# IIT-PAVIS/Acoustic-Image-Generation

Measured on AMD Instinct MI355X. Metric: train-step images/sec, higher is better.
Workload: dtype f32

## Files before the change

### acoustic-image-generation_amd/csrc/igemm.hip

```cpp
#include "wgrad_split3_kernel.hpp"
#include "wgrad_tap_kernel.hpp"
#include "igemm_split3d_kernel.hpp"
#include "igemm_split3dp_kernel.hpp"
#include "igemm_split3r_kernel.hpp"
#include "igemm_split3h_kernel.hpp"
#include "skinny_kernel.hpp"
#include <cstdlib>
#include <algorithm>
#include <type_traits>

namespace acimg {

__global__ __launch_bounds__(256) void igemm_splitk_reduce_kernel(const float* slab, int splits,
                                                                  int M, int Ngemm, int slab_ld,
                                                                  const EpiParams e) {
    const long idx = (long)blockIdx.x * 256 + threadIdx.x;
    const long total = (long)M * Ngemm;
    if (idx >= total) return;
    const int m = (int)(idx / Ngemm);
    const int n = (int)(idx - (long)m * Ngemm);
    float v = 0.f;
    for (int z = 0; z < splits; ++z) v += slab[((long)z * M + m) * slab_ld + n];
    if (n >= e.Nstore) return;
    int cn, pixoff, r, q, oh, ow;
    epi_col(e, n, cn, pixoff, r, q);
    const long rp = epi_row_pix(e, m, oh, ow);
    if (epi_lands(e, oh, ow, r, q)) epi_store(e, rp + pixoff, cn, v);
}

__global__ __launch_bounds__(256) void subpixel_weights_kernel(const float* w, int R, int S, int Ko, int Kin, int ldw, int U,
                                                               int V, float* wc, int total) {
    const int idx = blockIdx.x * 256 + threadIdx.x;
    if (idx >= total) return;
    const int ncol = 4 * Ko;
    const int row = idx / ncol, col = idx - row * ncol;
    const int kin = row % Kin, tap = row / Kin;
    const int up = tap / V, vp = tap - up * V;
    const int cls = col / Ko, ko = col - cls * Ko;
    const int a = cls >> 1, b = cls & 1;
    const int r = a + 2 * (U - 1 - up), q = b + 2 * (V - 1 - vp);
    wc[idx] = (r < R && q < S) ? w[((long)(r * S + q) * Ko + ko) * ldw + kin] : 0.f;
}

template <int BMO, int BN, int WGM = 2>
__global__ __launch_bounds__(256) void wgrad_f32_kernel(const WgradParams p) {
    constexpr int BKR = 16;
    constexpr int LDA_S = BMO + 4;
    constexpr int LDB_S = BN + 4;
    constexpr int WGN = 4 / WGM;
    constexpr int WTM = BMO / WGM, WTN = BN / WGN;
    static_assert(WTM % 16 == 0 && WTN % 16 == 0, "wave tile");
    constexpr int TM = WTM / 16, TN = WTN / 16;
    constexpr int AQ = BMO / 4;
    constexpr int ARPP = 256 / AQ;
    constexpr int NA = (BKR + ARPP - 1) / ARPP;
    constexpr int BQ = BN / 4;
    constexpr int BRPP = 256 / BQ;
    constexpr int NB = (BKR + BRPP - 1) / BRPP;

    __shared__ __attribute__((aligned(16))) float As[BKR * LDA_S];
    __shared__ __attribute__((aligned(16))) float Bs[BKR * LDB_S];

    const int tid = threadIdx.x;
    const int lane = tid & 63, wid = tid >> 6;
    const int wm = wid / WGN, wn = wid % WGN;
    const int li = lane & 15, g = lane >> 4;
    const int kk0 = blockIdx.x * BMO, n0 = blockIdx.y * BN;

    const int m_begin = blockIdx.z * p.rows_per_split;
    const int m_end = min(p.M, m_begin + p.rows_per_split);

    const int aq = tid % AQ;
    const int arow0 = tid / AQ;
    const int kk = kk0 + aq * 4;
    const bool kk_ok = kk < p.KK;
    const bool kk_ones = p.db_out != nullptr && kk == p.KK;
    int r = 0, s = 0, c = 0;
    if (kk_ok) {
        const int tap = kk / p.C;
        c = kk - tap * p.C;
        r = tap / p.S;
        s = tap - r * p.S;
    }
    const int bq = tid % BQ;
    const int brow0 = tid / BQ;
    const int nb = n0 + bq * 4;
    const bool nb_ok = nb < p.Nld;
    const int ohw = p.OH * p.OW;

    int x_img[NA], x_oh[NA], x_ow[NA];
#pragma unroll
    for (int j = 0; j < NA; ++j) {
        const int m = m_begin + arow0 + j * ARPP;
        x_img[j] = m / ohw;
        const int rem = m - x_img[j] * ohw;
        x_oh[j] = rem / p.OW;
        x_ow[j] = rem - x_oh[j] * p.OW;
    }

    float4 ra[NA], rb[NB];
    auto load_tiles = [&](int mb) {
#pragma unroll
        for (int j = 0; j < NA; ++j) {
            const int row = arow0 + j * ARPP;
            const int m = mb + row;
            float4 v = make_float4(0.f, 0.f, 0.f, 0.f);
            if (row < BKR && kk_ones && m < m_end) v.x = 1.f;
            if (row < BKR && kk_ok && m < m_end) {
                const int ih = x_oh[j] * p.stride - p.pad_t + r;
                const int iw = x_ow[j] * p.stride - p.pad_l + s;
                if ((unsigned)ih < (unsigned)p.H && (unsigned)iw < (unsigned)p.W)
                    v = *reinterpret_cast<const float4*>(
                        p.X + ((long)(x_img[j] * p.H + ih) * p.W + iw) * p.ldx + c);
            }
            ra[j] = v;
            x_ow[j] += BKR;
            while (x_ow[j] >= p.OW) {
                x_ow[j] -= p.OW;
                if (++x_oh[j] == p.OH) {
                    x_oh[j] = 0;
                    ++x_img[j];
                }
            }
        }
#pragma unroll
        for (int j = 0; j < NB; ++j) {
            const int row = brow0 + j * BRPP;
            const int m = mb + row;
            float4 v = make_float4(0.f, 0.f, 0.f, 0.f);
            if (row < BKR && nb_ok && m < m_end)
                v = *reinterpret_cast<const float4*>(p.G + (long)m * p.ldg + nb);
            rb[j] = v;
        }
    };
    auto store_tiles = [&]() {
#pragma unroll
        for (int j = 0; j < NA; ++j) {
            const int row = arow0 + j * ARPP;
            if (row < BKR) *reinterpret_cast<float4*>(&As[row * LDA_S + aq * 4]) = ra[j];
        }
#pragma unroll
        for (int j = 0; j < NB; ++j) {
            const int row = brow0 + j * BRPP;
            if (row < BKR) *reinterpret_cast<float4*>(&Bs[row * LDB_S + bq * 4]) = rb[j];
        }
    };

    f32x4 acc[TM][TN];
#pragma unroll
    for (int i = 0; i < TM; ++i)
#pragma unroll
        for (int j = 0; j < TN; ++j) acc[i][j] = f32x4{0.f, 0.f, 0.f, 0.f};

    if (m_begin < m_end) {
        load_tiles(m_begin);
        store_tiles();
    }
    __syncthreads();
    for (int mb = m_begin; mb < m_end; mb += BKR) {
        const bool more = (mb + BKR) < m_end;
        if (more) load_tiles(mb + BKR);
        float af[TM][4], bf[TN][4];
#pragma unroll
        for (int t = 0; t < 4; ++t) {
#pragma unroll
            for (int i = 0; i < TM; ++i) af[i][t] = As[(4 * g + t) * LDA_S + wm * WTM + i * 16 + li];
#pragma unroll
            for (int j = 0; j < TN; ++j) bf[j][t] = Bs[(4 * g + t) * LDB_S + wn * WTN + j * 16 + li];
        }
#pragma unroll
        for (int t = 0; t < 4; ++t)
#pragma unroll
            for (int i = 0; i < TM; ++i)
#pragma unroll
                for (int j = 0; j < TN; ++j)
                    acc[i][j] = __builtin_amdgcn_mfma_f32_16x16x4f32(af[i][t], bf[j][t], acc[i][j], 0, 0, 0);
        __syncthreads();
        if (more) {
            store_tiles();
            __syncthreads();
        }
    }

    float* out = p.out + (long)blockIdx.z * p.KK * p.ldo;
#pragma unroll
    for (int i = 0; i < TM; ++i)
#pragma unroll
        for (int rg = 0; rg < 4; ++rg) {
            const int row = kk0 + wm * WTM + i * 16 + g * 4 + rg;
            if (row > p.KK || (row == p.KK && p.db_out == nullptr)) continue;
            float* dst = row < p.KK ? out + (long)row * p.ldo : p.db_out + (long)blockIdx.z * p.ldo;
#pragma unroll
            for (int j = 0; j < TN; ++j) {
                const int n = n0 + wn * WTN + j * 16 + li;
                if (n < p.Ngemm) dst[n] = acc[i][j][rg];
            }
        }
}

__global__ __launch_bounds__(256) void slab_reduce_kernel(const float* slab, int splits, long rows,
                                                          int ncols, int ld, float* out, int nb1,
                                                          const float* slab2, float* out2) {
    long bid = blockIdx.x;
    if (bid >= nb1) {
        bid -= nb1;
        slab = slab2;
        out = out2;
        rows = 1;
    }
    const long idx = bid * 256 + threadIdx.x;
    if (idx >= rows * ncols) return;
    const long row = idx / ncols;
    const int col = (int)(idx - row * ncols);
    float v = 0.f;
    for (int z = 0; z < splits; ++z) v += slab[((long)z * rows + row) * ld + col];
    out[row * ld + col] = v;
}

template <int OUTS>
__global__ __launch_bounds__(256) void slab_reduce_wide_kernel(const float* slab, int splits, long rows,
                                                               int ncols, int ld, float* out, int nb1,
                                                               const float* slab2, float* out2) {
    constexpr int NG = 256 / OUTS;
    __shared__ float red[NG][OUTS];
    const int ol = threadIdx.x % OUTS, rg = threadIdx.x / OUTS;
    long bid = blockIdx.x;
    if (bid >= nb1) {
        bid -= nb1;
        slab = slab2;
        out = out2;
        rows = 1;
    }
    const long idx = bid * OUTS + ol;
    const bool ok = idx < rows * ncols;
    const long row = ok ? idx / ncols : 0;
    const int col = ok ? (int)(idx - row * ncols) : 0;
    const float* src = slab + row * ld + col;
    const long zs = rows * ld;
    float v0 = 0.f, v1 = 0.f, v2 = 0.f, v3 = 0.f;
    if (ok) {
        int z = rg;
        for (; z + 3 * NG < splits; z += 4 * NG) {
            v0 += src[(long)z * zs];
            v1 += src[(long)(z + NG) * zs];
            v2 += src[(long)(z + 2 * NG) * zs];
            v3 += src[(long)(z + 3 * NG) * zs];
        }
        for (; z < splits; z += NG) v0 += src[(long)z * zs];
    }
    red[rg][ol] = (v0 + v1) + (v2 + v3);
    __syncthreads();
    if (rg == 0 && ok) {
        float t = 0.f;
#pragma unroll
        for (int i = 0; i < NG; ++i) t += red[i][ol];
        out[row * ld + col] = t;
    }
}
static void launch_slab_reduce_wide(const float* slab, int splits, long rows, int ncols, int ld, float* out, const float* slab2,
                                    float* out2, hipStream_t st) {
    const long total = rows * ncols;
    if (total <= 4096) {
        const int nb1 = (int)cdiv(total, 8), nb2 = out2 ? cdiv(ncols, 8) : 0;
        hipLaunchKernelGGL(slab_reduce_wide_kernel<8>, dim3(nb1 + nb2), dim3(256), 0, st, slab, splits, rows, ncols, ld, out, nb1,
                           slab2, out2);
    } else {
        const int nb1 = (int)cdiv(total, 32), nb2 = out2 ? cdiv(ncols, 32) : 0;
        hipLaunchKernelGGL(slab_reduce_wide_kernel<32>, dim3(nb1 + nb2), dim3(256), 0, st, slab, splits, rows, ncols, ld, out, nb1,
                           slab2, out2);
    }
}

__global__ __launch_bounds__(256) void tapconv_pack_kernel(const float* w, int taps, int C, int K, int ldw,
                                                           float* wt, int ldwt) {
    const long idx = (long)blockIdx.x * 256 + threadIdx.x;
    const int TK = taps * K;
    if (idx >= (long)C * TK) return;
    const int c = (int)(idx / TK), n = (int)(idx - (long)c * TK);
    const int tap = n / K, k = n - tap * K;
    wt[(long)c * ldwt + n] = w[((long)tap * C + c) * ldw + k];
}

__global__ __launch_bounds__(256) void tapconv_unpack_kernel(const float* dwt, int ldwt, int taps, int C, int K,
                                                             int ldw, const float* w, float decay, float* dw) {
    const long idx = (long)blockIdx.x * 256 + threadIdx.x;
    if (idx >= (long)taps * C * K) return;
    const int k = (int)(idx % K);
    const long tc = idx / K;
    const int c = (int)(tc % C), tap = (int)(tc / C);
    float v = dwt[(long)c * ldwt + tap * K + k];
    if (w) v = fmaf(decay, w[tc * ldw + k], v);
    dw[tc * ldw + k] = v;
}

constexpr int TG_PPB = 32;
__global__ __launch_bounds__(256) void tapconv_gather_kernel(const float* z, int ldz, int H, int W, int R, int S,
                                                             int K, int OH, int OW, long Mout, float* y, int ldy,
                                                             float* stats, int stats_ld) {
    extern __shared__ __attribute__((aligned(16))) float tg_smem[];
    const int ppb = TG_PPB;
    const long m0 = (long)blockIdx.x * ppb;
    for (int e = threadIdx.x; e < ppb * K; e += 256) {
        const int pl = e / K, k = e - pl * K;
        const long m = m0 + pl;
// ... 1674 lines not shown
    float* Y; int ldy, nout;
    const float* bias; const float* res; int ldres; const float* mask; int ldmask;
    float* stats; int stats_ld;
    int tiles_x, tiles_y; long tiles;
};

template <typename TR, int TERMS, int CIN, int NOUT, int MODE>
__global__ __launch_bounds__(512, 1) void conv_halo16_kernel(const ConvHaloParams p) {
    typedef typename TR::V8 V8;
    constexpr int TH = TERMS == 1 ? 8 : 4, TW = 32, XH = TH + 2, XWV = TW + 2, XW = 36;
    constexpr int PITCH = CIN * 2 + 16;
    constexpr int XPL = XH * XW * PITCH;
    constexpr int KTOT = 9 * CIN;
    constexpr int WROW = KTOT * 2 + 16;
    constexpr int WPL = NOUT * WROW;
    constexpr int NPL = TERMS == 3 ? 2 : 1;
    constexpr int MT = TERMS == 1 ? 2 : 1;
    constexpr int NT = NOUT / 16;
    constexpr int NXL = (XH * XWV * (CIN / 4) + 511) / 512;
    extern __shared__ __attribute__((aligned(16))) float ch16_smem[];
    char* const xl = reinterpret_cast<char*>(ch16_smem);
    char* const wl = xl + NPL * XPL;
    const int tid = threadIdx.x, lane = tid & 63, wid = tid >> 6;
    const int li = lane & 15, g = lane >> 4;
    const int jrow = TERMS == 1 ? wid : wid >> 1;
    const int mcol0 = TERMS == 1 ? 0 : (wid & 1) * 16;

    for (int i = tid; i < NPL * NOUT * (KTOT / 8); i += 512) {
        const int ch = i % (KTOT / 8), r2 = i / (KTOT / 8);
        const int n = r2 % NOUT, pl = r2 / NOUT;
        const uint4 v = *reinterpret_cast<const uint4*>(p.Wimg + (size_t)pl * p.w_lo_off + ((size_t)n * KTOT + ch * 8) * 2);
        *reinterpret_cast<uint4*>(wl + pl * WPL + n * WROW + ch * 16) = v;
    }

    float4 rx[NXL];
    unsigned okm = 0;
    const float4 asc = p.a_scale ? *reinterpret_cast<const float4*>(p.a_scale + (tid % (CIN / 4)) * 4) : make_float4(1.f, 1.f, 1.f, 1.f);
    const float4 ash = p.a_scale ? *reinterpret_cast<const float4*>(p.a_shift + (tid % (CIN / 4)) * 4) : make_float4(0.f, 0.f, 0.f, 0.f);
    auto load_tile = [&](long tile) {
        okm = 0;
        const int tx = (int)(tile % p.tiles_x);
        const long t2 = tile / p.tiles_x;
        const int ty = (int)(t2 % p.tiles_y);
        const long img = t2 / p.tiles_y;
        const float* xi = p.X + img * p.H * p.W * p.ldx;
#pragma unroll
        for (int k = 0; k < NXL; ++k) {
            const int i = tid + 512 * k;
            const int c4 = i % (CIN / 4), pix = i / (CIN / 4);
            const int row = pix / XWV, col = pix - row * XWV;
            const int iy = ty * TH + row - 1, ix = tx * TW + col - 1;
            float4 v = make_float4(0.f, 0.f, 0.f, 0.f);
            if (row < XH && (unsigned)iy < (unsigned)p.H && (unsigned)ix < (unsigned)p.W) {
                v = *reinterpret_cast<const float4*>(xi + ((long)iy * p.W + ix) * p.ldx + c4 * 4);
                okm |= 1u << k;
            }
            rx[k] = v;
        }
    };
    auto store_tile = [&]() {
#pragma unroll
        for (int k = 0; k < NXL; ++k) {
            const int i = tid + 512 * k;
            const int c4 = i % (CIN / 4), pix = i / (CIN / 4);
            const int row = pix / XWV, col = pix - row * XWV;
            if (row < XH) {
                const int off = (row * XW + col) * PITCH + c4 * 8;
                uint2 hi, lo;
                split4<TR>(p.a_scale && ((okm >> k) & 1u) ? affine_relu4(rx[k], asc, ash, p.a_relu != 0) : rx[k], hi, lo);
                *reinterpret_cast<uint2*>(xl + off) = hi;
                if (TERMS == 3) *reinterpret_cast<uint2*>(xl + XPL + off) = lo;
            }
        }
    };

    f32x4 s1[NT], s2[NT];
#pragma unroll
    for (int n = 0; n < NT; ++n) s1[n] = s2[n] = f32x4{0.f, 0.f, 0.f, 0.f};
    f32x4 bv[NT];
#pragma unroll
    for (int n = 0; n < NT; ++n)
        bv[n] = (MODE == 0 && p.bias) ? *reinterpret_cast<const f32x4*>(p.bias + n * 16 + 4 * g) : f32x4{0.f, 0.f, 0.f, 0.f};

    const int a_base = (jrow * XW + mcol0 + li) * PITCH + g * 16;
    const int b_base = li * WROW + g * 16;

    long tile = blockIdx.x;
    if (tile < p.tiles) load_tile(tile);
    for (; tile < p.tiles; tile += gridDim.x) {
        __syncthreads();
        store_tile();
        __syncthreads();
        const int tx = (int)(tile % p.tiles_x);
        const long t2 = tile / p.tiles_x;
        const int ty = (int)(t2 % p.tiles_y);
        const long img = t2 / p.tiles_y;
        if (tile + gridDim.x < p.tiles) load_tile(tile + gridDim.x);
        f32x4 acc[MT][NT];
#pragma unroll
        for (int m = 0; m < MT; ++m)
#pragma unroll
            for (int n = 0; n < NT; ++n) acc[m][n] = f32x4{0.f, 0.f, 0.f, 0.f};
#pragma unroll
        for (int r = 0; r < 3; ++r)
#pragma unroll
            for (int s_ = 0; s_ < 3; ++s_)
#pragma unroll
                for (int ck = 0; ck < CIN / 32; ++ck) {
                    V8 ah[MT], al[MT], bh[NT], bl[NT];
#pragma unroll
                    for (int m = 0; m < MT; ++m) {
                        const int off = a_base + (r * XW + s_ + 16 * m) * PITCH + ck * 64;
                        ah[m] = *reinterpret_cast<const V8*>(xl + off);
                        if (TERMS == 3) al[m] = *reinterpret_cast<const V8*>(xl + XPL + off);
                    }
#pragma unroll
                    for (int n = 0; n < NT; ++n) {
                        const int off = b_base + n * 16 * WROW + ((r * 3 + s_) * CIN + ck * 32) * 2;
                        bh[n] = *reinterpret_cast<const V8*>(wl + off);
                        if (TERMS == 3) bl[n] = *reinterpret_cast<const V8*>(wl + WPL + off);
                    }
#pragma unroll
                    for (int m = 0; m < MT; ++m)
#pragma unroll
                        for (int n = 0; n < NT; ++n) {
                            if (TERMS == 3) {
                                acc[m][n] = TR::mfma(bl[n], ah[m], acc[m][n]);
                                acc[m][n] = TR::mfma(bh[n], al[m], acc[m][n]);
                            }
                            acc[m][n] = TR::mfma(bh[n], ah[m], acc[m][n]);
                        }
                }
        const int oy = ty * TH + jrow;
#pragma unroll
        for (int m = 0; m < MT; ++m) {
            const int ox = tx * TW + mcol0 + 16 * m + li;
            if (oy < p.H && ox < p.W) {
                const long pix = (img * p.H + oy) * p.W + ox;
#pragma unroll
                for (int n = 0; n < NT; ++n) {
                    if (NOUT == 16 && n * 16 + 4 * g >= p.nout) continue;
                    f32x4 v = acc[m][n] * TR::OUTSCALE + bv[n];
                    if (MODE == 1) {
                        if (p.res) v += *reinterpret_cast<const f32x4*>(p.res + pix * p.ldres + n * 16 + 4 * g);
                        if (p.mask) {
                            const f32x4 k = *reinterpret_cast<const f32x4*>(p.mask + pix * p.ldmask + n * 16 + 4 * g);
#pragma unroll
                            for (int c = 0; c < 4; ++c) v[c] = k[c] > 0.f ? v[c] : 0.f;
                        }
                    } else {
                        s1[n] += v;
                        s2[n] += v * v;
                    }
                    *reinterpret_cast<f32x4*>(p.Y + pix * p.ldy + n * 16 + 4 * g) = v;
                }
            }
        }
    }
    if (MODE == 0 && p.stats) {
        __syncthreads();
        float* red = reinterpret_cast<float*>(xl);
#pragma unroll
        for (int n = 0; n < NT; ++n)
#pragma unroll
            for (int c = 0; c < 4; ++c) {
                const float a = row16_sum(s1[n][c]), b = row16_sum(s2[n][c]);
                if (li == 0) {
                    red[(wid * 2 + 0) * NOUT + n * 16 + 4 * g + c] = a;
                    red[(wid * 2 + 1) * NOUT + n * 16 + 4 * g + c] = b;
                }
            }
        __syncthreads();
        if (tid < 2 * NOUT) {
            const int which = tid / NOUT, n = tid % NOUT;
            float t = 0.f;
#pragma unroll
            for (int w = 0; w < 8; ++w) t += red[(w * 2 + which) * NOUT + n];
            p.stats[((long)blockIdx.x * 2 + which) * p.stats_ld + n] = t;
        }
    }
}

static bool conv_halo16_fwd_shape(const AcimgConvDesc* d) {
    return d->R == 3 && d->S == 3 && d->stride == 1 && d->pad_t == 1 && d->pad_l == 1 && d->OH == d->H && d->OW == d->W &&
           (d->C == 32 || d->C == 64) && d->K == 32 && (long)d->N * d->H * d->W >= 65536 && d->act == ACIMG_ACT_NONE &&
           g_cfg.wgrad_halo;
}
static bool conv_halo16_dgrad_shape(const AcimgConvDesc* d) {
    return d->R == 3 && d->S == 3 && d->stride == 1 && d->pad_t == 1 && d->pad_l == 1 && d->OH == d->H && d->OW == d->W &&
           (d->C == 32 || d->C == 64) && d->K == 32 && (long)d->N * d->H * d->W >= 65536 && g_cfg.wgrad_halo;
}
static constexpr int CONV_HALO16_WGS = 256;

template <typename TR, int TERMS, int CIN, int NOUT, int MODE>
static int launch_conv_halo16(ConvHaloParams q, int N, hipStream_t st) {
    constexpr int TH = TERMS == 1 ? 8 : 4, NPL = TERMS == 3 ? 2 : 1;
    constexpr int lds = NPL * ((TH + 2) * 36 * (CIN * 2 + 16) + NOUT * (9 * CIN * 2 + 16));
    static_assert(lds <= 160 * 1024 && 8 * 2 * NOUT * 4 <= lds, "LDS budget");
    q.tiles_x = cdiv(q.W, 32); q.tiles_y = cdiv(q.H, TH);
    q.tiles = (long)N * q.tiles_x * q.tiles_y;
    if (!q.nout) q.nout = NOUT;
    static bool attr_set = false;
    if (!attr_set) {
        (void)hipFuncSetAttribute(reinterpret_cast<const void*>(conv_halo16_kernel<TR, TERMS, CIN, NOUT, MODE>),
                                  hipFuncAttributeMaxDynamicSharedMemorySize, lds);
        attr_set = true;
    }
    hipLaunchKernelGGL((conv_halo16_kernel<TR, TERMS, CIN, NOUT, MODE>), dim3(CONV_HALO16_WGS), dim3(512), lds, st, q);
    return check_launch("conv_halo16");
}

static int dgrad_halo16_narrow(const AcimgConvDesc* d, const float* gy, int ldgy, const float* w, float* dx, int lddx,
                               const float* residual, int ldres, const float* mask, int ldmask, void* ws, hipStream_t st) {
    FewParams f{};
    f.w = w; f.ldw = d->ldw; f.wrows = d->C; f.cin = d->K; f.mode = 1; f.nout = d->C;
    hipLaunchKernelGGL((few16_prepare_kernel<SplitBF16>), dim3(cdiv(16 * 288, 256)), dim3(256), 0, st, f, 32, 16,
                       static_cast<__bf16*>(ws));
    ConvHaloParams q{};
    q.X = gy; q.H = d->H; q.W = d->W; q.ldx = ldgy; q.Wimg = static_cast<const char*>(ws); q.w_lo_off = 16 * 288 * 2;
    q.Y = dx; q.ldy = lddx; q.nout = d->C; q.res = residual; q.ldres = ldres; q.mask = mask; q.ldmask = ldmask;
    return launch_conv_halo16<SplitBF16, 3, 32, 16, 1>(q, d->N, st);
}

enum TrunkKind { TRUNK_ONE_TILE = 0, TRUNK_PERSISTENT = 1, TRUNK_RING = 2, TRUNK_HALO = 3 };
struct TrunkPick {
    TrunkKind kind;
    int bm, bn;
    int stats_rows;
    bool big_out;
};

static constexpr int HALO_NB = 18;
static bool halo_applies(const AcimgConvDesc* d, int terms, const Split3Cfg& c) {
    if (terms != 3 || d->R != 3 || d->S != 3 || d->stride != 1 || d->pad_t != 1 || d->pad_l != 1 || d->OH != d->H ||
        d->OW != d->W || d->C % 32)
        return false;
    if (c.bm != 128 || c.bn != 128) return false;
    return ((d->W + 16) >> 4) + 8 + (d->W >> 4) + 1 <= HALO_NB;
}

static TrunkPick pick_trunk(const AcimgConvDesc* d, int terms, bool two_pass) {
    const int M = d->N * d->OH * d->OW;
    const Split3Cfg c = pick_split3(M, d->K);
    const bool t128 = c.bm == 128 && c.bn == 128;
    TrunkPick t{TRUNK_ONE_TILE, c.bm, c.bn, 0, (long)M * d->ldy * 4 >= (1L << 31)};
    if (two_pass) t.kind = TRUNK_PERSISTENT;
    else if (g_cfg.trunk_halo == 2 && halo_applies(d, terms, c)) t.kind = TRUNK_HALO;
    int ring_rows = 0;
    if (!two_pass && t.kind != TRUNK_HALO && !t.big_out && g_cfg.trunk_ring && terms == 3 && t128) {
        const long t128s = (long)cdiv(M, 128) * cdiv(d->K, 128);
        const int kiters = d->R * d->S * (d->C / 32);
        const long t256 = (long)cdiv(M, 256) * cdiv(d->K, 128);
        if (g_cfg.trunk_ring == 1) ring_rows = (t128s > 256 && t128s <= 300 && kiters >= 64) ? 128 : 0;
        else if (g_cfg.trunk_ring_bm) ring_rows = g_cfg.trunk_ring_bm;
        else ring_rows = t256 >= 500 ? 256 : 128;
    }
    if (ring_rows) {
        t.kind = TRUNK_RING;
        t.bm = ring_rows;
    }
    const long tiles = (long)cdiv(M, c.bm) * cdiv(d->K, c.bn);
    if (t.kind == TRUNK_ONE_TILE && !t.big_out && t128 && (g_cfg.trunk_persistent == 2 || (g_cfg.trunk_persistent == 1 && tiles >= 512)))
        t.kind = TRUNK_PERSISTENT;
    t.stats_rows = cdiv(M, t.bm);
    return t;
}

static size_t split3_rowmajor_bytes(const AcimgConvDesc* d) { return (size_t)2 * d->ldw * d->R * d->S * d->C * 2; }
static size_t split3_brick_bytes(const AcimgConvDesc* d) {
    return d->C % 32 ? 0 : (size_t)cdiv(d->ldw, 128) * (d->R * d->S * d->C / 32) * 2 * 8192;
}
__global__ void split3_brick_kernel(const char* __restrict__ planes, char* __restrict__ bricks, const int Nrows,
                                    const int Ktot, const long total) {
    const long i = (long)blockIdx.x * 256 + threadIdx.x;
    if (i >= total) return;
    const int pch = (int)(i & 3), row = (int)((i >> 2) & 127), plane = (int)((i >> 9) & 1);
    const long bq = i >> 10;
    const int kit = Ktot / 32;
    const int nt = (int)(bq / kit), q = (int)(bq - (long)nt * kit);
    const int n = nt * 128 + row;
    uint4 v = make_uint4(0, 0, 0, 0);
    if (n < Nrows)
        v = *reinterpret_cast<const uint4*>(planes + (((long)plane * Nrows + n) * Ktot + q * 32 + ((pch ^ swz(row)) << 3)) * 2);
    *reinterpret_cast<uint4*>(bricks + i * 16) = v;
}

template <typename TR, int TERMS = 3>
static int launch_split3(IgemmParams& p, hipStream_t st) {
    Split3Cfg c = pick_split3(p.M, p.Ngemm, true);
    dim3 grid(cdiv(p.M, c.bm), cdiv(p.Ngemm, c.bn), 1);
    if (c.bm == 128 && c.bn == 32)
        hipLaunchKernelGGL((igemm_split3_kernel<128, 32, 4, 1, 256, TR, TERMS>), grid, dim3(256), 2 * (2 * 128 * 64 + 2 * 32 * 64), st, p);
    else if (c.bm == 128 && c.bn == 128)
        hipLaunchKernelGGL((igemm_split3_kernel<128, 128, 2, 4, 512, TR, TERMS>), grid, dim3(512), 65536, st, p);
    else if (c.bm == 64 && c.bn == 128)
        hipLaunchKernelGGL((igemm_split3_kernel<64, 128, 1, 4, 256, TR, TERMS>), grid, dim3(256), 2 * (2 * 64 * 64 + 2 * 128 * 64), st, p);
    else if (c.bm == 128 && c.bn == 64)
        hipLaunchKernelGGL((igemm_split3_kernel<128, 64, 2, 2, 256, TR, TERMS>), grid, dim3(256), 2 * (2 * 128 * 64 + 2 * 64 * 64), st, p);
    else
        return fail(ACIMG_EINVAL, "split3: unsupported tile %dx%d", c.bm, c.bn);
    return check_launch("igemm_split3");
}

static int fwd_split_onthefly(const AcimgConvDesc* d, const float* x, const void* wsplit, const float* bias, float* y,
                              const float* in_scale, const float* in_shift, int in_relu, float* stats, void* stream,
                              bool bf16) {
    int rc = check_desc(d, "conv2d_fwd_split3", true);
    if (rc) return rc;
    if (d->C % 32) return fail(ACIMG_EINVAL, "conv2d_fwd_split3: C=%d must be a multiple of 32", d->C);
    if (d->ldw < d->K || !aligned16(x) || !aligned16(wsplit))
        return fail(ACIMG_EINVAL, "conv2d_fwd_split3: ldw<K or unaligned operands");
    if (conv_halo16_fwd_shape(d)) {
        if ((in_scale != nullptr) != (in_shift != nullptr) || (in_relu && !in_scale) || !aligned16(y) || (d->ldy & 3) || (d->ldx & 3) ||
            (bias && !aligned16(bias)) || (in_scale && (!aligned16(in_scale) || !aligned16(in_shift))))
            return fail(ACIMG_EINVAL, "conv2d_fwd_split3: the halo form of this shape needs scale AND shift of an input affine, "
                                      "16-byte aligned y / bias / affine and ldx, ldy multiples of 4");
        ConvHaloParams q{};
        q.a_scale = in_scale; q.a_shift = in_shift; q.a_relu = in_relu;
        q.X = x; q.H = d->H; q.W = d->W; q.ldx = d->ldx; q.Wimg = static_cast<const char*>(wsplit);
        q.w_lo_off = (unsigned)((size_t)d->ldw * d->R * d->S * d->C * 2);
        q.Y = y; q.ldy = d->ldy; q.bias = bias; q.stats = stats; q.stats_ld = d->ldw;
        hipStream_t st = (hipStream_t)stream;
        if (bf16) return d->C == 64 ? launch_conv_halo16<SplitBF16, 1, 64, 32, 0>(q, d->N, st)
                                    : launch_conv_halo16<SplitBF16, 1, 32, 32, 0>(q, d->N, st);
        return d->C == 64 ? launch_conv_halo16<SplitF16, 3, 64, 32, 0>(q, d->N, st)
                          : launch_conv_halo16<SplitF16, 3, 32, 32, 0>(q, d->N, st);
    }
    IgemmParams p = fwd_view(d);
    split_ksteps(p);
    p.A = x; p.a_scale = in_scale; p.a_shift = in_shift; p.a_relu = in_relu;
    p.B = static_cast<const float*>(wsplit);
    const long a_bytes = (((long)d->N * d->H * d->W - 1) * d->ldx + d->C) * 4;
    const long b_bytes = (long)acimg_conv2d_split3_weight_bytes(d);
    if (a_bytes >= (1L << 31) || b_bytes >= (1L << 31)) return fail(ACIMG_EINVAL, "conv2d_fwd_split3: operand >= 2 GiB");
    p.a_bytes = (unsigned)a_bytes; p.b_bytes = (unsigned)b_bytes;
    p.e.Y = y; p.e.bias = bias; p.e.stats = stats;
    epi_vec_flag(p.e);
    if (bf16) return launch_split3<SplitBF16, 1>(p, (hipStream_t)stream);
    return launch_split3<SplitF16>(p, (hipStream_t)stream);
}

static int dgrad_split_onthefly(const AcimgConvDesc* d, const float* gy, int ldgy, const void* wsplit_t, float* dx,
                                int lddx, const float* residual, int ldres, const float* mask, int ldmask,
                                void* stream, int terms) {
    int rc = check_desc(d, "conv2d_dgrad_split3");
    if (rc) return rc;
    if (d->stride != 1 || d->K % 32 || d->K > ldgy || (ldgy & 3))
        return fail(ACIMG_EINVAL, "conv2d_dgrad_split3: needs stride 1 and K %% 32 == 0 (K=%d)", d->K);
    if (lddx <= 0) lddx = d->ldx;
    if (conv_halo16_dgrad_shape(d) && aligned16(gy) && aligned16(wsplit_t) && aligned16(dx) && (lddx & 3) == 0 &&
        (!residual || (aligned16(residual) && (ldres & 3) == 0)) && (!mask || (aligned16(mask) && (ldmask & 3) == 0))) {
        ConvHaloParams q{};
        q.X = gy; q.H = d->H; q.W = d->W; q.ldx = ldgy; q.Wimg = static_cast<const char*>(wsplit_t);
        q.w_lo_off = (unsigned)((size_t)d->C * d->R * d->S * d->K * 2);
        q.Y = dx; q.ldy = lddx; q.res = residual; q.ldres = ldres; q.mask = mask; q.ldmask = ldmask;
        hipStream_t st = (hipStream_t)stream;
        if (terms == 1) return d->C == 64 ? launch_conv_halo16<SplitBF16, 1, 32, 64, 1>(q, d->N, st)
                                          : launch_conv_halo16<SplitBF16, 1, 32, 32, 1>(q, d->N, st);
        return d->C == 64 ? launch_conv_halo16<SplitBF16, 3, 32, 64, 1>(q, d->N, st)
                          : launch_conv_halo16<SplitBF16, 3, 32, 32, 1>(q, d->N, st);
    }
    IgemmParams p = flipped_view(d, d->K, ldgy);
    split_ksteps(p);
    p.A = gy; p.B = static_cast<const float*>(wsplit_t); p.Nld = d->C;
    const long a_bytes = (((long)d->N * d->OH * d->OW - 1) * ldgy + d->K) * 4;
    const long b_bytes = (long)acimg_conv2d_split3_dgrad_weight_bytes(d);
    if (a_bytes >= (1L << 31) || b_bytes >= (1L << 31)) return fail(ACIMG_EINVAL, "conv2d_dgrad_split3: operand >= 2 GiB");
    p.a_bytes = (unsigned)a_bytes; p.b_bytes = (unsigned)b_bytes;
    EpiParams& e = p.e;
    e.Y = dx; e.ldy = lddx; e.res = residual; e.ldres = ldres; e.mask = mask; e.ldmask = ldmask;
    epi_vec_flag(e);
    if (terms == 1) return launch_split3<SplitBF16, 1>(p, (hipStream_t)stream);
    return launch_split3<SplitBF16>(p, (hipStream_t)stream);
}

struct TailPlan { int whole, s, rem; };

struct TrunkVariant {
    const void* fn;
    int threads;
    size_t lds;
    int wgs_per_cu;
    bool lds_opt_in;
    TrunkVariant* slots_of;
    int slots;
    bool opted_in;
};
static constexpr size_t tile_lds(size_t bm, size_t bn) { return std::max(2 * 2 * (bm + bn) * 64, bm * bn * 4) + 4 * 2 * bn * 4; }
static constexpr size_t PERSISTENT_LDS = (size_t)2 * 4 * 128 * 64 + 4 * 2 * 128 * 4;
static constexpr size_t ring_lds(size_t rows) { return 3 * 2 * (rows + 128) * 64 + 4 * 2 * 128 * 4; }
static constexpr size_t HALO_LDS = (size_t)2 * (HALO_NB * 1024 + 64) + 2 * 2 * 128 * 64;
#define ACIMG_KFN(...) reinterpret_cast<const void*>(__VA_ARGS__)
static TrunkVariant TILE_128x128 = {ACIMG_KFN(igemm_split3d_kernel<128, 128, 2, 4, 512, 2, 2>), 512, tile_lds(128, 128), 2, false, nullptr};
static TrunkVariant TILE_64x128 = {ACIMG_KFN(igemm_split3d_kernel<64, 128, 1, 4, 256, 2, 2>), 256, tile_lds(64, 128), 3, false, nullptr};
static TrunkVariant TILE_128x64 = {ACIMG_KFN(igemm_split3d_kernel<128, 64, 2, 2, 256, 2, 2>), 256, tile_lds(128, 64), 3, false, nullptr};
static TrunkVariant TILE1_128x128 = {ACIMG_KFN(igemm_split3d_kernel<128, 128, 2, 4, 512, 2, 2, 1>), 512, tile_lds(128, 128), 2, false, &TILE_128x128};
static TrunkVariant TILE1_64x128 = {ACIMG_KFN(igemm_split3d_kernel<64, 128, 1, 4, 256, 2, 2, 1>), 256, tile_lds(64, 128), 3, false, &TILE_64x128};
static TrunkVariant TILE1_128x64 = {ACIMG_KFN(igemm_split3d_kernel<128, 64, 2, 2, 256, 2, 2, 1>), 256, tile_lds(128, 64), 3, false, &TILE_128x64};
static TrunkVariant PERSISTENT = {ACIMG_KFN(igemm_split3dp_kernel<32, 0>), 512, PERSISTENT_LDS, 2, false, nullptr};
static TrunkVariant PERSISTENT_SPREAD = {ACIMG_KFN(igemm_split3dp_kernel<32, 1>), 512, PERSISTENT_LDS, 2, false, &PERSISTENT};
static TrunkVariant PERSISTENT1 = {ACIMG_KFN(igemm_split3dp_kernel<32, 0, 1>), 512, PERSISTENT_LDS, 2, false, &PERSISTENT};
static TrunkVariant PASS_STATS = {ACIMG_KFN(igemm_split3dp_kernel<32, 0, 3, 1>), 512, PERSISTENT_LDS, 2, false, nullptr};
static TrunkVariant PASS_TAIL = {ACIMG_KFN(igemm_split3dp_kernel<32, 0, 3, 2>), 512, PERSISTENT_LDS, 2, false, nullptr};
static TrunkVariant PASS_TAIL_PROJ = {ACIMG_KFN(igemm_split3dp_kernel<32, 0, 3, 3>), 512, PERSISTENT_LDS, 2, false, nullptr};
static TrunkVariant RING_256 = {ACIMG_KFN(igemm_split3r_kernel<4>), 512, ring_lds(256), 1, true, nullptr};
static TrunkVariant RING_128 = {ACIMG_KFN(igemm_split3r_kernel<2>), 512, ring_lds(128), 1, true, nullptr};
static TrunkVariant HALO = {ACIMG_KFN(igemm_split3h_kernel<HALO_NB>), 512, HALO_LDS, 2, true, nullptr};
#undef ACIMG_KFN

static void opt_in_lds(TrunkVariant& v) {
    if (!v.lds_opt_in || v.opted_in) return;
    (void)hipFuncSetAttribute(v.fn, hipFuncAttributeMaxDynamicSharedMemorySize, (int)v.lds);
    v.opted_in = true;
}
static int resident_slots(TrunkVariant& v) {
    opt_in_lds(v);
    TrunkVariant& o = v.slots_of ? *v.slots_of : v;
    if (!o.slots) {
        int dev = 0, ncu = 0, per = 0;
        if (hipGetDevice(&dev) != hipSuccess ||
            hipDeviceGetAttribute(&ncu, hipDeviceAttributeMultiprocessorCount, dev) != hipSuccess ||
            hipOccupancyMaxActiveBlocksPerMultiprocessor(&per, o.fn, o.threads, v.lds) != hipSuccess || ncu <= 0 || per <= 0) {
            (void)hipGetLastError();
            ncu = 256;
            per = o.wgs_per_cu;
        }
        o.slots = ncu * per;
    }
    return o.slots;
}
static void launch_trunk(const TrunkVariant& v, int nwg, hipStream_t st, IgemmParams& p, int units = 0, int cap = 0) {
    void* args[] = {&p, &units, &cap};
    (void)hipLaunchKernel(v.fn, dim3(nwg), dim3(v.threads), args, v.lds, st);
}
static TailPlan pick_tail(int T, int P, int KI, int max_units) {
    const int rem = T % P;
    TailPlan best{T, 1, 0};
    if (rem == 0 || !g_cfg.tail_split) return best;
    if (g_cfg.tail_s) {
        const int s = g_cfg.tail_s;
        if (s > 1 && KI / s >= 1 && (long)rem * s <= max_units) return TailPlan{T - rem, s, rem};
        return best;
    }
    double best_cost = KI;
    static const int cand[] = {2, 3, 4, 6, 8, 12, 16};
    for (int s : cand) {
        if (KI / s < 2 || (long)rem * s > max_units) break;
        const double cost = (double)cdiv((long)rem * s, P) * cdiv(KI, s) + 8.0 + 1.0 * s;
        if (cost < 0.9 * best_cost) {
            best_cost = cost;
            best = TailPlan{T - rem, s, rem};
        }
    }
    return best;
}
static constexpr int TS_MAX_UNITS = 1024;
static constexpr size_t TS_COUNTER_BYTES = 4096;
static constexpr size_t TS_WS_BYTES = TS_COUNTER_BYTES + (size_t)TS_MAX_UNITS * 128 * 128 * sizeof(float);

static int wire_tail(IgemmParams& p, void* ws, size_t ws_bytes, int tiles, int slots, int max_units, bool allow) {
    TailPlan t{tiles, 1, 0};
    if (allow && ws && ws_bytes >= TS_WS_BYTES) t = pick_tail(tiles, slots, p.kiters, max_units);
    p.ts_whole = t.whole; p.ts_s = t.s;
    p.ts_counters = static_cast<int*>(ws);
    p.ts_partial = ws ? reinterpret_cast<float*>(static_cast<char*>(ws) + TS_COUNTER_BYTES) : nullptr;
    return t.whole + t.rem * t.s;
}

#if defined(ACIMG_STAMP) || defined(ACIMG_ABLATE)
static float* g_stamp_buf = nullptr;
static int g_stamp_nostore = 0;
#endif

struct Split3pTail {
    int mode;
    const float* scale;
    const float* shift;
    const void* sc_planes;
    size_t sc_lo_off;
    void* out_planes;
    size_t out_lo_off;
    const float* scale2;
    const float* shift2;
};

static int fwd_presplit(const AcimgConvDesc* d, const void* x_planes, size_t x_lo_off, const void* wsplit, float* y,
                        float* stats, void* ws, size_t ws_bytes, void* stream, const int terms,
                        const Split3pTail* tail = nullptr) {
    int rc = check_desc(d, "conv2d_fwd_split3p");
    if (rc) return rc;
    if (d->C % 32) return fail(ACIMG_EINVAL, "conv2d_fwd_split3p: C=%d must be a multiple of 32", d->C);
    if (d->ldw < d->K || !aligned16(x_planes) || !aligned16(wsplit) || !aligned16(y) || (d->ldy & 3) || d->ldx != d->C ||
        (x_lo_off & 15))
        return fail(ACIMG_EINVAL, "conv2d_fwd_split3p: ldw<K, ldx != C (split-format tensors are dense) or unaligned operands");
    IgemmParams p = fwd_view(d);
    split_ksteps(p);
    p.A = static_cast<const float*>(x_planes); p.B = static_cast<const float*>(wsplit);
    const long plane = (long)acimg_split_plane_bytes((long)d->N * d->H * d->W, d->C);
    const long a_bytes = (long)x_lo_off + plane;
    const long b_bytes = (long)acimg_conv2d_split3_weight_bytes(d);
    if (a_bytes >= (1L << 31) || b_bytes >= (1L << 31) || (long)x_lo_off < plane)
        return fail(ACIMG_EINVAL, "conv2d_fwd_split3p: operand >= 2 GiB or overlapping planes");
    p.a_bytes = (unsigned)a_bytes; p.b_bytes = (unsigned)b_bytes; p.a_lo_off = (unsigned)x_lo_off;
    p.b_brick = (unsigned)split3_rowmajor_bytes(d);
    EpiParams& e = p.e;
    e.Y = y; e.stats = stats; e.vec = 1;
    const TrunkPick t = pick_trunk(d, terms, tail != nullptr);
    hipStream_t st = (hipStream_t)stream;
    p.ras_tiles_m = cdiv(p.M, t.bm);
    p.ras_tiles_n = cdiv(d->K, t.bn);
    p.ras_gn = std::min(p.ras_tiles_n, 8);
    p.ras_gm = std::max(1, (t.kind == TRUNK_RING ? 32 : 64) / p.ras_gn);
    const int T = p.ras_tiles_m * p.ras_tiles_n;
    const bool t128 = t.bm == 128 && t.bn == 128;
    if (tail) {
        if (terms != 3 || !t128 || t.big_out || d->K % 128 || d->ldy != d->K || d->ldw != d->K)
            return fail(ACIMG_EINVAL, "conv2d_fwd_split3p (two-pass): needs 128x128 tiles, K %% 128 == 0, dense output < 2 GiB");
        TrunkVariant& v = tail->mode == 1 ? PASS_STATS : tail->mode == 2 ? PASS_TAIL : PASS_TAIL_PROJ;
        const int slots = resident_slots(v);
        const int units = wire_tail(p, ws, ws_bytes, T, slots, TS_MAX_UNITS, true);
        const int nwg = std::min(units, slots);
        const char* what = "conv2d_fwd_split3p_stats";
        e.Y = nullptr;
        if (tail->mode != 1) {
            const long oplane = (long)acimg_split_plane_bytes((long)p.M, d->K);
            if (!aligned16(tail->sc_planes) || !aligned16(tail->out_planes) || (tail->out_lo_off & 15) ||
                (long)tail->out_lo_off < oplane || (long)tail->out_lo_off + oplane >= (1L << 31))
                return fail(ACIMG_EINVAL, "conv2d_fwd_split3p_tail: unaligned / overlapping / >= 2 GiB split-format operands");
            e.stats = nullptr;
            e.f_scale = tail->scale; e.f_shift = tail->shift;
            e.f_sc = static_cast<const char*>(tail->sc_planes);
            e.f_out = static_cast<char*>(tail->out_planes); e.f_out_lo = (unsigned)tail->out_lo_off;
            e.f_out_bytes = (unsigned)(tail->out_lo_off + oplane);
            if (tail->mode == 3) {
                e.f_scale2 = tail->scale2; e.f_shift2 = tail->shift2;
                e.f_sc_lo = 0; e.f_sc_bytes = (unsigned)((long)p.M * d->K * 4);
                what = "conv2d_fwd_split3p_tail_proj";
            } else {
                if ((tail->sc_lo_off & 15) || (long)tail->sc_lo_off < oplane || (long)tail->sc_lo_off + oplane >= (1L << 31))
                    return fail(ACIMG_EINVAL, "conv2d_fwd_split3p_tail: unaligned / overlapping / >= 2 GiB shortcut planes");
                e.f_sc_lo = (unsigned)tail->sc_lo_off;
                e.f_sc_bytes = (unsigned)(tail->sc_lo_off + oplane);
                what = "conv2d_fwd_split3p_tail";
            }
        }
        launch_trunk(v, nwg, st, p, units, nwg);
        return check_launch(what);
    }
    if (t.kind == TRUNK_HALO) {
        const int units = wire_tail(p, ws, ws_bytes, T, resident_slots(HALO), TS_MAX_UNITS, true);
        launch_trunk(HALO, units, st, p);
        return check_launch("conv2d_fwd_split3p (halo)");
    }
#if defined(ACIMG_STAMP) || defined(ACIMG_ABLATE)
    p.slab = g_stamp_buf;
    p.flip = g_stamp_nostore;
#endif
    if (t.kind == TRUNK_RING) {
        TrunkVariant& v = t.bm == 256 ? RING_256 : RING_128;
        const int slots = resident_slots(v);
        const int units = wire_tail(p, ws, ws_bytes, T, slots, TS_MAX_UNITS * 128 / t.bm, true);
        const int nwg = std::min(units, slots);
        p.splits = g_cfg.trunk_stagger > 0 ? 2 : 1;
        launch_trunk(v, nwg, st, p, units, nwg);
        return check_launch("conv2d_fwd_split3p (ring)");
    }
    if (t.kind == TRUNK_PERSISTENT) {
        TrunkVariant& v = terms == 1 ? PERSISTENT1 : g_cfg.trunk_dma_pos == 1 ? PERSISTENT_SPREAD : PERSISTENT;
        const int slots = resident_slots(v);
        const int units = wire_tail(p, ws, ws_bytes, T, slots, TS_MAX_UNITS, true);
        p.splits = g_cfg.trunk_stagger > 0 ? g_cfg.trunk_stagger * (p.kiters * 2500 + 8000) / 100 : 1;
        const int nwg = std::min(units, slots);
        launch_trunk(v, nwg, st, p, units, nwg);
        return check_launch("conv2d_fwd_split3p");
    }
    TrunkVariant& v = t128 ? (terms == 1 ? TILE1_128x128 : TILE_128x128)
                    : t.bm == 64 ? (terms == 1 ? TILE1_64x128 : TILE_64x128) : (terms == 1 ? TILE1_128x64 : TILE_128x64);
    const int units = wire_tail(p, ws, ws_bytes, T, resident_slots(v), TS_MAX_UNITS, t128);
    launch_trunk(v, units, st, p);
    return check_launch("conv2d_fwd_split3p");
}

static int tapconv_check(const AcimgConvDesc* d, const char* who) {
    int rc = check_desc(d, who);
    if (rc) return rc;
    if (d->stride != 1 || d->pad_t || d->pad_l || d->OH != d->H - d->R + 1 || d->OW != d->W - d->S + 1)
        return fail(ACIMG_EINVAL, "%s: stride-1 VALID convolutions only", who);
    if (d->K > 64) return fail(ACIMG_EINVAL, "%s: K=%d > 64 (this form is for few output channels)", who, d->K);
    return ACIMG_OK;
}

static int wgrad_split_onthefly(const AcimgConvDesc* d, const float* x, const float* gy, int ldgy, float* dw, float* db,
                                void* ws, size_t ws_bytes, void* stream, int terms) {
    int rc = check_desc(d, "conv2d_wgrad_split3");
    if (rc) return rc;
    const int kp = up4(d->K);
    if (kp > ldgy || kp > d->ldw) return fail(ACIMG_EINVAL, "conv2d_wgrad_split3: padded K exceeds ldgy/ldw");
    WgradParams p{};
    p.X = x; p.H = d->H; p.W = d->W; p.C = d->C; p.ldx = d->ldx;
    p.OH = d->OH; p.OW = d->OW; p.R = d->R; p.S = d->S; p.stride = d->stride; p.pad_t = d->pad_t; p.pad_l = d->pad_l;
    p.M = d->N * d->OH * d->OW; p.KK = d->R * d->S * d->C;
    p.G = gy; p.ldg = ldgy; p.Ngemm = kp; p.Nld = kp; p.ldo = d->ldw;
    return launch_wgrad(p, dw, db, ws, ws_bytes, (hipStream_t)stream, true, terms);
}

}

using namespace acimg;

extern "C" {

int acimg_conv2d_stats_rows(const AcimgConvDesc* d) {
    if (few16_fwd_shape(d)) return FEW16_WGS;
    return cdiv((long)d->N * d->OH * d->OW, stats_block_rows(d));
}

int acimg_conv2d_fwd_tiling(const AcimgConvDesc* d, int* out) {
    if (!d || !out) return fail(ACIMG_EINVAL, "conv2d_fwd_tiling: null argument");
    const int M = d->N * d->OH * d->OW;
    TileCfg c = pick_cfg(M, d->K);
    out[0] = c.bm;
    out[1] = c.bn;
    out[2] = pick_splits(M, d->K, c, fwd_kiters(d));
    return ACIMG_OK;
}

int acimg_config_default(AcimgConfig* c) {
    if (!c) return fail(ACIMG_EINVAL, "config_default: null");
    *c = AcimgConfig{320, 768, 1, 128, 1, 0, 0, 1, 0, 1, 0, 0, 0, 1, 0, 0};
    return ACIMG_OK;
}

int acimg_configure(const AcimgConfig* c) {
    if (!c) return fail(ACIMG_EINVAL, "configure: null");
    if (c->splitk_cut < 0 || c->splitk_target < 1 || c->wgrad_minpix < 1 || c->tail_s < 0)
        return fail(ACIMG_EINVAL, "configure: negative / zero tuning value");
    if (c->trunk_persistent < 0 || c->trunk_persistent > 2) return fail(ACIMG_EINVAL, "configure: trunk_persistent is 0, 1 or 2");
    if (c->trunk_dma_pos < 0 || c->trunk_dma_pos > 1) return fail(ACIMG_EINVAL, "configure: trunk_dma_pos is 0 or 1");
    if (c->trunk_stagger < 0 || c->trunk_stagger > 100) return fail(ACIMG_EINVAL, "configure: trunk_stagger is a percentage");
    if (c->trunk_bk != 0 && c->trunk_bk != 32)
        return fail(ACIMG_EINVAL, "configure: trunk_bk must be 0 or 32 (the 64-deep K step was measured slower and removed)");
    if (c->trunk_ring < 0 || c->trunk_ring > 2) return fail(ACIMG_EINVAL, "configure: trunk_ring is 0, 1 or 2");
    if (c->trunk_ring_bm != 0 && c->trunk_ring_bm != 128 && c->trunk_ring_bm != 256)
        return fail(ACIMG_EINVAL, "configure: trunk_ring_bm must be 0 (per shape), 128 or 256");
    if (c->trunk_halo < 0 || c->trunk_halo > 2) return fail(ACIMG_EINVAL, "configure: trunk_halo is 0, 1 or 2");
    if (c->split3_tile_bm || c->split3_tile_bn) {
        const int bm = c->split3_tile_bm, bn = c->split3_tile_bn;
        if (!((bm == 128 && bn == 128) || (bm == 64 && bn == 128) || (bm == 128 && bn == 64)))
            return fail(ACIMG_EINVAL, "configure: split3 tile %dx%d is not an instantiated tile", bm, bn);
    }
    g_cfg = *c;
    return ACIMG_OK;
}

size_t acimg_conv2d_fwd_workspace(const AcimgConvDesc* d) {
    const size_t a = igemm_ws_bytes(d->N * d->OH * d->OW, d->K, fwd_kiters(d));
    const size_t b = direct_shape(d->C, d->K) ? direct_ws_bytes(d->R, d->S, d->C, (d->K + 7) & ~7) : 0;
    const size_t c = skinny_fwd_ws_bytes(d);
    const size_t f = few16_fwd_shape(d) ? few16_ws_bytes(d->C, d->K) : 0;
    return std::max(std::max(a, f), std::max(b, c));
}

int acimg_conv2d_fwd(const AcimgConvDesc* d, const float* x, const float* w, const float* bias,
                     float* y, const float* in_scale, const float* in_shift, int in_relu,
                     float* stats, void* ws, size_t ws_bytes, void* tickets, void* stream) {
    int rc = check_desc(d, "conv2d_fwd");
    if (rc) return rc;
    if (d->ldw < d->K) return fail(ACIMG_EINVAL, "conv2d_fwd: ldw < K");
    if (skinny_shape(d) && !in_scale && !in_shift && !in_relu && !stats && ws && ws_bytes >= skinny_fwd_ws_bytes(d) && aligned16(x) &&
        aligned16(w) && aligned16(y) && aligned16(ws) && (!bias || aligned16(bias)) && (d->ldw & 3) == 0 && (d->ldx & 3) == 0 &&
        (d->ldy & 3) == 0) {
        SkinnyParams q{};
        q.W = w; q.X = x; q.out = y; q.bias = bias; q.act = d->act; q.part = static_cast<float*>(ws);
        q.M = d->N; q.C = d->C; q.N = d->K; q.ldw = d->ldw; q.ldx = d->ldx; q.ldo = d->ldy;
// ... 593 lines not shown
```

Before: 4959.

## Add tap-wise halo conv kernel for 3x3 stride-1 convs on 32/48-wide images

Adds a new implicit-GEMM kernel that stages a two-row input halo tile (split into hi/lo halves) in LDS once per 32-channel slice, then iterates over the nine filter taps and reads shifted windows from that tile. The input is no longer gathered again for every tap, and weight loads are double-buffered. It is dispatched for forward and dgrad 3x3 convolutions with width 32 or 48, C>=64, three split terms, no input affine and no stats. It adds a new code path with its own tile sizes and LDS footprint, and it could have lower occupancy than the existing split3 kernels.

```diff
diff --git a/acoustic-image-generation_amd/csrc/conv_tap_kernel.hpp b/acoustic-image-generation_amd/csrc/conv_tap_kernel.hpp
--- /dev/null
+++ b/acoustic-image-generation_amd/csrc/conv_tap_kernel.hpp
@@ -0,0 +1,169 @@
+#pragma once
+#include "igemm_split3_kernel.hpp"
+
+namespace acimg {
+
+constexpr int CT_TH = 2, CT_PITCH = 64;
+static constexpr int conv_tap_lds(int W, int NB) { return 2 * (CT_TH + 2) * (W + 2) * CT_PITCH + 2 * 2 * NB * 64; }
+
+template <typename TR, int W, int NB>
+__global__ __launch_bounds__(512, 4) void conv_tap_kernel(const IgemmParams p) {
+    typedef typename TR::V8 V8;
+    constexpr int TH = CT_TH, XH = TH + 2, XW = W + 2, PITCH = CT_PITCH;
+    constexpr int XPL = XH * XW * PITCH;
+    constexpr int BM = TH * W, WGM = TH, WGN = 8 / WGM, WTM = BM / WGM, WTN = NB / WGN, TM = WTM / 16, TN = WTN / 16;
+    constexpr int B_BYTES = NB * 64, WSTAGE = 2 * B_BYTES;
+    constexpr int NXL = (XH * XW * 8 + 511) / 512;
+    constexpr int NBL = 2 * NB * 4 / 512;
+    static_assert((NB == 128 || NB == 64) && W % 16 == 0 && WTM == W && XPL % 16 == 0, "tile / thread mapping");
+
+    extern __shared__ __attribute__((aligned(16))) float smem[];
+    char* const lds = reinterpret_cast<char*>(smem);
+    char* const wst = lds + 2 * XPL;
+
+    const int tid = threadIdx.x, lane = tid & 63, wid = tid >> 6;
+    const int wm = wid / WGN, wn = wid % WGN;
+    const int li = lane & 15, g = lane >> 4;
+    const int tiles_y = (p.H + TH - 1) / TH;
+    const int img = blockIdx.x / tiles_y, y0 = (blockIdx.x - img * tiles_y) * TH;
+    const int m0 = (img * p.H + y0) * W, n0 = blockIdx.y * NB;
+    const int Ktot = 9 * p.C;
+
+    const __amdgpu_buffer_rsrc_t rsA =
+        __builtin_amdgcn_make_buffer_rsrc(const_cast<float*>(p.A), 0, p.a_bytes, 0x00020000);
+    const __amdgpu_buffer_rsrc_t rsB =
+        __builtin_amdgcn_make_buffer_rsrc(const_cast<float*>(p.B), 0, p.b_bytes, 0x00020000);
+
+    const int x_lds0 = (tid >> 3) * PITCH + (((tid >> 1) & 3) ^ (2 * ((tid >> 5) & 1))) * 16 + (tid & 1) * 8;
+    unsigned x_voff[NXL];
+#pragma unroll
+    for (int k = 0; k < NXL; ++k) {
+        const int pix = (tid >> 3) + 64 * k;
+        const int row = pix / XW, col = pix - row * XW;
+        const bool ok = row < XH && col >= 1 && col <= W && (unsigned)(y0 + row - 1) < (unsigned)p.H;
+        x_voff[k] = ok ? (unsigned)(((m0 + (row - 1) * W + col - 1) * p.lda + (tid & 7) * 4) * 4) : OOB;
+    }
+    const int b_which = tid / (NB * 4), b_row = (tid & (NB * 4 - 1)) >> 2, b_kc = tid & 3;
+    const unsigned b_plane = (unsigned)((long)p.Nld * Ktot * 2);
+    const unsigned b_goff0 = n0 + b_row < p.Nld ? (unsigned)((((long)b_which * p.Nld + n0 + b_row) * Ktot + b_kc * 8) * 2) : OOB;
+    const int b_lds0 = b_which * B_BYTES + b_row * 64 + ((b_kc ^ swz(b_row)) << 4);
+
+    float4 rx[NXL];
+    uint4 rb0[NBL], rb1[NBL];
+    const int n_it = 9 * (p.C >> 5);
+    int nit = 0, ld_tap = 0, ld_c0 = 0;
+    int xc0 = 0;
+
+    auto load_x = [&]() {
+#pragma unroll
+        for (int k = 0; k < NXL; ++k)
+            rx[k] = __builtin_bit_cast(float4, __builtin_amdgcn_raw_buffer_load_b128(rsA, x_voff[k], xc0 * 4, 0));
+        xc0 += 32;
+    };
+    auto store_x = [&]() {
+#pragma unroll
+        for (int k = 0; k < NXL; ++k) {
+            if ((tid >> 3) + 64 * k < XH * XW) {
+                uint2 hi, lo;
+                split4<TR>(rx[k], hi, lo);
+                *reinterpret_cast<uint2*>(lds + x_lds0 + 64 * k * PITCH) = hi;
+                *reinterpret_cast<uint2*>(lds + XPL + x_lds0 + 64 * k * PITCH) = lo;
+            }
+        }
+    };
+    auto load_w = [&](uint4 (&rb)[NBL]) {
+        const int kbyte = (ld_tap * p.C + ld_c0) * 2;
+#pragma unroll
+        for (int j = 0; j < NBL; ++j)
+            rb[j] = __builtin_bit_cast(uint4, __builtin_amdgcn_raw_buffer_load_b128(
+                                                  rsB, b_goff0 == OOB ? OOB : b_goff0 + j * b_plane, kbyte, 0));
+        ++nit;
+        if (++ld_tap == 9) {
+            ld_tap = 0;
+            ld_c0 += 32;
+        }
+    };
+    auto store_w = [&](int buf, const uint4 (&rb)[NBL]) {
+#pragma unroll
+        for (int j = 0; j < NBL; ++j) *reinterpret_cast<uint4*>(wst + buf * WSTAGE + b_lds0 + j * B_BYTES) = rb[j];
+    };
+
+    f32x4 acc[TM][TN];
+#pragma unroll
+    for (int i = 0; i < TM; ++i)
+#pragma unroll
+        for (int j = 0; j < TN; ++j) acc[i][j] = f32x4{0.f, 0.f, 0.f, 0.f};
+
+    const int a_pix = wm * XW + li;
+    const int b_off = (wn * WTN + li) * 64 + ((g ^ swz(li)) << 4);
+    auto compute = [&](int buf, int tap) {
+        const int r = (tap * 11) >> 5, s = tap - 3 * r;
+        const int px = a_pix + r * XW + s;
+        const char* xa = lds + px * PITCH + ((g ^ (2 * ((px >> 2) & 1))) << 4);
+        const char* wb = wst + buf * WSTAGE;
+        V8 ah[TM], al[TM], bh[TN], bl[TN];
+#pragma unroll
+        for (int i = 0; i < TM; ++i) {
+            ah[i] = *reinterpret_cast<const V8*>(xa + i * 16 * PITCH);
+            al[i] = *reinterpret_cast<const V8*>(xa + XPL + i * 16 * PITCH);
+        }
+#pragma unroll
+        for (int j = 0; j < TN; ++j) {
+            bh[j] = *reinterpret_cast<const V8*>(wb + b_off + j * 16 * 64);
+            bl[j] = *reinterpret_cast<const V8*>(wb + B_BYTES + b_off + j * 16 * 64);
+        }
+        __builtin_amdgcn_sched_barrier(0);
+#pragma unroll
+        for (int i = 0; i < TM; ++i)
+#pragma unroll
+            for (int j = 0; j < TN; ++j) acc[i][j] = TR::mfma(bl[j], ah[i], acc[i][j]);
+#pragma unroll
+        for (int i = 0; i < TM; ++i)
+#pragma unroll
+            for (int j = 0; j < TN; ++j) acc[i][j] = TR::mfma(bh[j], al[i], acc[i][j]);
+#pragma unroll
+        for (int i = 0; i < TM; ++i)
+#pragma unroll
+            for (int j = 0; j < TN; ++j) acc[i][j] = TR::mfma(bh[j], ah[i], acc[i][j]);
+    };
+
+    int tp = 0;
+    auto advance = [&](int buf, uint4 (&rb)[NBL], int it) {
+        if (it + 1 < n_it) {
+            if (tp == 8) {
+                __syncthreads();
+                store_x();
+                if (xc0 < p.C) load_x();
+            }
+            store_w(buf, rb);
+            if (nit < n_it) load_w(rb);
+        }
+        __syncthreads();
+        tp = tp == 8 ? 0 : tp + 1;
+    };
+
+    load_x();
+    load_w(rb0);
+    store_x();
+    store_w(0, rb0);
+    if (xc0 < p.C) load_x();
+    if (nit < n_it) load_w(rb0);
+    if (nit < n_it) load_w(rb1);
+    __syncthreads();
+    for (int it = 0; it < n_it; it += 2) {
+        compute(0, tp);
+        advance(1, rb0, it);
+        if (it + 1 >= n_it) break;
+        compute(1, tp);
+        advance(0, rb1, it + 1);
+    }
+
+#pragma unroll
+    for (int i = 0; i < TM; ++i)
+#pragma unroll
+        for (int j = 0; j < TN; ++j)
+            if (TR::OUTSCALE != 1.f) acc[i][j] *= TR::OUTSCALE;
+    if (y0 + wm < p.H) igemm_epilogue<BM, NB, WGM, WGN, 512, TM, TN>(p, acc, smem, m0, n0, wm, wn, li, g, tid);
+}
+
+}
diff --git a/acoustic-image-generation_amd/csrc/igemm.hip b/acoustic-image-generation_amd/csrc/igemm.hip
--- a/acoustic-image-generation_amd/csrc/igemm.hip
+++ b/acoustic-image-generation_amd/csrc/igemm.hip
@@ -1,5 +1,6 @@
 #include "wgrad_split3_kernel.hpp"
 #include "wgrad_tap_kernel.hpp"
+#include "conv_tap_kernel.hpp"
 #include "igemm_split3d_kernel.hpp"
 #include "igemm_split3dp_kernel.hpp"
 #include "igemm_split3r_kernel.hpp"
@@ -2280,6 +2281,21 @@
     return check_launch("igemm_split3");
 }
 
+static bool conv_tap_ok(const IgemmParams& p, int terms) {
+    return terms == 3 && p.R == 3 && p.S == 3 && p.stride == 1 && p.pad_t == 1 && p.pad_l == 1 && p.OH == p.H && p.OW == p.W &&
+           (p.W == 32 || p.W == 48) && p.C >= 64 && p.C % 32 == 0 && p.Ngemm > 32 && p.e.vec && (p.lda & 3) == 0 &&
+           aligned16(p.A) && aligned16(p.B) && p.M % (p.H * p.W) == 0 && !p.a_scale && !p.e.stats && p.splits == 1 && g_cfg.wgrad_halo;
+}
+template <typename TR>
+static int launch_conv_tap(const IgemmParams& p, hipStream_t st) {
+    const dim3 grid(p.M / (p.H * p.W) * cdiv(p.H, CT_TH), cdiv(p.Ngemm, p.Ngemm <= 64 ? 64 : 128), 1);
+#define ACIMG_CT(Wv, NBv) hipLaunchKernelGGL((conv_tap_kernel<TR, Wv, NBv>), grid, dim3(512), conv_tap_lds(Wv, NBv), st, p)
+    if (p.W == 48) { if (p.Ngemm <= 64) ACIMG_CT(48, 64); else ACIMG_CT(48, 128); }
+    else           { if (p.Ngemm <= 64) ACIMG_CT(32, 64); else ACIMG_CT(32, 128); }
+#undef ACIMG_CT
+    return check_launch("conv_tap");
+}
+
 static int fwd_split_onthefly(const AcimgConvDesc* d, const float* x, const void* wsplit, const float* bias, float* y,
                               const float* in_scale, const float* in_shift, int in_relu, float* stats, void* stream,
                               bool bf16) {
@@ -2314,6 +2330,7 @@
     p.a_bytes = (unsigned)a_bytes; p.b_bytes = (unsigned)b_bytes;
     p.e.Y = y; p.e.bias = bias; p.e.stats = stats;
     epi_vec_flag(p.e);
+    if (conv_tap_ok(p, bf16 ? 1 : 3)) return launch_conv_tap<SplitF16>(p, (hipStream_t)stream);
     if (bf16) return launch_split3<SplitBF16, 1>(p, (hipStream_t)stream);
     return launch_split3<SplitF16>(p, (hipStream_t)stream);
 }
@@ -2348,6 +2365,7 @@
     EpiParams& e = p.e;
     e.Y = dx; e.ldy = lddx; e.res = residual; e.ldres = ldres; e.mask = mask; e.ldmask = ldmask;
     epi_vec_flag(e);
+    if (conv_tap_ok(p, terms)) return launch_conv_tap<SplitBF16>(p, (hipStream_t)stream);
     if (terms == 1) return launch_split3<SplitBF16, 1>(p, (hipStream_t)stream);
     return launch_split3<SplitBF16>(p, (hipStream_t)stream);
 }
```

New measurement: 5071 (median of 6 runs). 1.02x the previous value.
